# orishu/kraken

Hardware: AMD Instinct MI355X
Metric: metainfo+digest GB/s (device-resident & end-to-end) at 1/2/4/8 MI355X (higher is better)
Workload: dtype u8

## Files before the change

kraken_amd/csrc/sha256_multi.hip:

```cpp
#include <stdlib.h>

#include <atomic>
#include <mutex>
#include <type_traits>

#include "../../include/kraken_hip_internal.h"
#include "kernels.hpp"
#include "knobs.hpp"
#include "device_util.hpp"

namespace krk {

#define KRK_K256                                                                                 \
    0x428a2f98u, 0x71374491u, 0xb5c0fbcfu, 0xe9b5dba5u, 0x3956c25bu, 0x59f111f1u, 0x923f82a4u,     \
        0xab1c5ed5u, 0xd807aa98u, 0x12835b01u, 0x243185beu, 0x550c7dc3u, 0x72be5d74u, 0x80deb1feu, \
        0x9bdc06a7u, 0xc19bf174u, 0xe49b69c1u, 0xefbe4786u, 0x0fc19dc6u, 0x240ca1ccu, 0x2de92c6fu, \
        0x4a7484aau, 0x5cb0a9dcu, 0x76f988dau, 0x983e5152u, 0xa831c66du, 0xb00327c8u, 0xbf597fc7u, \
        0xc6e00bf3u, 0xd5a79147u, 0x06ca6351u, 0x14292967u, 0x27b70a85u, 0x2e1b2138u, 0x4d2c6dfcu, \
        0x53380d13u, 0x650a7354u, 0x766a0abbu, 0x81c2c92eu, 0x92722c85u, 0xa2bfe8a1u, 0xa81a664bu, \
        0xc24b8b70u, 0xc76c51a3u, 0xd192e819u, 0xd6990624u, 0xf40e3585u, 0x106aa070u, 0x19a4c116u, \
        0x1e376c08u, 0x2748774cu, 0x34b0bcb5u, 0x391c0cb3u, 0x4ed8aa4au, 0x5b9cca4fu, 0x682e6ff3u, \
        0x748f82eeu, 0x78a5636fu, 0x84c87814u, 0x8cc70208u, 0x90befffau, 0xa4506cebu, 0xbef9a3f7u, \
        0xc67178f2u

// ... 216 lines not shown
            const int i = 4 * q + t;
            uint32_t wi;
            if (i < 16) {
                wi = w[i];
            } else {
                const uint32_t w15 = w[(i - 15) & 15], w2 = w[(i - 2) & 15];
                const uint32_t s0 = xor3(rotr(w15, 7), rotr(w15, 18), w15 >> 3);
                const uint32_t s1 = xor3(rotr(w2, 17), rotr(w2, 19), w2 >> 10);
                wi = w[i & 15] + s0 + w[(i - 7) & 15] + s1;
                w[i & 15] = wi;
            }
            kw[t] = wi + K[i];
        }
        *reinterpret_cast<u32x4*>(lds + base + 256 * q) = u32x4{kw[0], kw[1], kw[2], kw[3]};
    }
}

template <int kNs, int kStep, bool kNoLoad = false>
__device__ __forceinline__ void produce_step(const ShaJob& job, uint32_t b, uint32_t ob, uint32_t nb,
                                             uint32_t col, uint32_t* lds, const u32x4 use[kRaw],
                                             u32x4 next[kRaw], uint64_t safe, uint32_t& passed) {
    const bool act = b < nb;
    if (act) {
        while (passed + kNs / kStep < b / kStep + 2) {
            __syncthreads();
            ++passed;
        }
    }
    if (kNoLoad) {
#pragma unroll
        for (int c = 0; c < kRaw; ++c) next[c] = u32x4{b, col, (uint32_t)c, b ^ col};
    } else {
        fetch(job, ob + 2 * kStep, next, safe);
    }
    const uint32_t base = kw_base((ob / kStep) % (kNs / kStep), col);
    if (act) build<kNs>(job, ob, use, base, lds);
}

#define KRK_SHA_ROUND(A, B, C, D, E, F, G, HK, KWN, NE, NA, NH)                  \
    "v_alignbit_b32 %[r6], %[" #E "], %[" #E "], 6\n\t"                        \
    "v_alignbit_b32 %[r11], %[" #E "], %[" #E "], 11\n\t"                      \
    "v_alignbit_b32 %[r25], %[" #E "], %[" #E "], 25\n\t"                      \
    "v_bitop3_b32 %[ch], %[" #E "], %[" #F "], %[" #G "] bitop3:0xca\n\t"     \
    "v_bitop3_b32 %[r6], %[r6], %[r11], %[r25] bitop3:0x96\n\t"                \
    "v_alignbit_b32 %[q2], %[" #A "], %[" #A "], 2\n\t"                        \
    "v_add3_u32 %[t1], %[" #HK "], %[r6], %[ch]\n\t"                           \
    "v_alignbit_b32 %[q13], %[" #A "], %[" #A "], 13\n\t"                      \
    "v_add_u32_e32 %[" #NE "], %[" #D "], %[t1]\n\t"                           \
    "v_alignbit_b32 %[q22], %[" #A "], %[" #A "], 22\n\t"                      \
    "v_bitop3_b32 %[mj], %[" #A "], %[" #B "], %[" #C "] bitop3:0xe8\n\t"     \
    "v_bitop3_b32 %[q2], %[q2], %[q13], %[q22] bitop3:0x96\n\t"                \
    "v_add_u32_e32 %[" #NH "], %[" #G "], %[" #KWN "]\n\t"                     \
    "v_add3_u32 %[" #NA "], %[t1], %[q2], %[mj]\n\t"

__device__ __forceinline__ void sha_quad(uint32_t& a, uint32_t& b, uint32_t& c, uint32_t& d, uint32_t& e,
                                         uint32_t& f, uint32_t& g, uint32_t& hk, uint32_t k1, uint32_t k2,
                                         uint32_t k3, uint32_t k4, uint32_t& h_last) {
    uint32_t r6, r11, r25, ch, q2, t1, q13, q22, mj;
    uint32_t e1, e2, e3, e4, a1, a2, a3, a4, h1, h2, h3, h4;
    asm volatile(KRK_SHA_ROUND(a, b, c, d, e, f, g, hk, k1, e1, a1, h1)
                 KRK_SHA_ROUND(a1, a, b, c, e1, e, f, h1, k2, e2, a2, h2)
                 KRK_SHA_ROUND(a2, a1, a, b, e2, e1, e, h2, k3, e3, a3, h3)
                 KRK_SHA_ROUND(a3, a2, a1, a, e3, e2, e1, h3, k4, e4, a4, h4)
                 : [r6] "=&v"(r6), [r11] "=&v"(r11), [r25] "=&v"(r25), [ch] "=&v"(ch), [q2] "=&v"(q2),
                   [t1] "=&v"(t1), [q13] "=&v"(q13), [q22] "=&v"(q22), [mj] "=&v"(mj), [e1] "=&v"(e1),
                   [e2] "=&v"(e2), [e3] "=&v"(e3), [e4] "=&v"(e4), [a1] "=&v"(a1), [a2] "=&v"(a2),
                   [a3] "=&v"(a3), [a4] "=&v"(a4), [h1] "=&v"(h1), [h2] "=&v"(h2), [h3] "=&v"(h3),
                   [h4] "=&v"(h4)
                 : [a] "v"(a), [b] "v"(b), [c] "v"(c), [d] "v"(d), [e] "v"(e), [f] "v"(f), [g] "v"(g),
                   [hk] "v"(hk), [k1] "v"(k1), [k2] "v"(k2), [k3] "v"(k3), [k4] "v"(k4));
    h_last = e1;
    a = a4; b = a3; c = a2; d = a1;
    e = e4; f = e3; g = e2;
    hk = h4;
}
#undef KRK_SHA_ROUND

__device__ __forceinline__ void rounds(uint32_t h[8], const uint32_t* lds, int slot, uint32_t lane,
                                       const u32x4& k0, const u32x4& k1) {
    uint32_t a = h[0], b = h[1], c = h[2], d = h[3], e = h[4], f = h[5], g = h[6];
    uint32_t hk = h[7] + k0[0], hl = 0;
    u32x4 kw = k0, nkw = k1, nnkw = k1;
#pragma unroll
    for (int q = 0; q < 16; ++q) {
        if (q + 2 < 16) nnkw = *reinterpret_cast<const u32x4*>(lds + kw_index(slot, q + 2, lane));
        sha_quad(a, b, c, d, e, f, g, hk, kw[1], kw[2], kw[3], q + 1 < 16 ? nkw[0] : 0u, hl);
        kw = nkw;
        nkw = nnkw;
    }
    h[0] += a; h[1] += b; h[2] += c; h[3] += d; h[4] += e; h[5] += f; h[6] += g; h[7] += hl;
}

__device__ __forceinline__ u32x4 kw_quad(const uint32_t* lds, int slot, int q, uint32_t lane) {
    return *reinterpret_cast<const u32x4*>(lds + kw_index(slot, q, lane));
}

__device__ __forceinline__ bool two_lane_is_e(uint32_t lane) { return (lane >> 3) & 1; }
__device__ __forceinline__ uint32_t two_lane_stream(uint32_t lane) {
    return (lane >> 4) * 8 + (two_lane_is_e(lane) ? 7 - (lane & 7) : (lane & 7));
}

#define KRK_SHA2_ROUND(X0, X1, X2, NX, WN)                                              \
    "v_add_u32_dpp %[p], %[" #X1 "], %[z] row_mirror row_mask:0xf bank_mask:0xf\n\t"    \
    "v_alignbit_b32 %[t1], %[" #X0 "], %[" #X0 "], %[r1]\n\t"                          \
    "v_alignbit_b32 %[t2], %[" #X0 "], %[" #X0 "], %[r2]\n\t"                          \
    "v_alignbit_b32 %[t3], %[" #X0 "], %[" #X0 "], %[r3]\n\t"                          \
    "v_bitop3_b32 %[k], %[" #X0 "], %[" #X1 "], %[ma] bitop3:0x2d\n\t"                 \
    "v_bitop3_b32 %[t1], %[t1], %[t2], %[t3] bitop3:0x96\n\t"                          \
    "v_bitop3_b32 %[k], %[k], %[" #X2 "], %[" #X1 "] bitop3:0xca\n\t"                  \
    "v_xad_u32 %[z], %[" #X2 "], %[ma], %[" #WN "]\n\t"                                \
    "v_add3_u32 %[" #NX "], %[t1], %[k], %[p]\n\t"

struct TwoLaneConst {
    uint32_t r1, r2, r3, ma;
};

#define KRK_SHA2_OPERANDS                                                                             \
    : [t1] "=&v"(t1), [t2] "=&v"(t2), [t3] "=&v"(t3), [k] "=&v"(kk), [p] "=&v"(p), [z] "+v"(z),       \
      [R0] "+v"(R0), [R1] "+v"(R1), [R2] "+v"(R2), [R3] "+v"(R3)
#define KRK_SHA2_CONSTS [r1] "v"(c.r1), [r2] "v"(c.r2), [r3] "v"(c.r3), [ma] "v"(c.ma)

#define KRK_SHA8_ROUND(X0, X1, X2, NX, WN) KRK_SHA8_ROUND_(X0, X1, X2, NX, "%[" #WN "]")
#define KRK_SHA8_ROUND_(X0, X1, X2, NX, W)                                                   \
    "v_alignbit_b32 %[t1], %[" #X0 "], %[" #X0 "], %[r1]\n\t"                               \
    "v_bitop3_b32 %[k], %[" #X0 "], %[" #X1 "], %[ma] bitop3:0x2d\n\t"                      \
    "v_bitop3_b32 %[k], %[k], %[" #X2 "], %[" #X1 "] bitop3:0xca\n\t"                       \
    "v_xor_b32_dpp %[t2], %[t1], %[t1] quad_perm:[1,2,0,3] row_mask:0xf bank_mask:0xf\n\t"  \
    "v_xor_b32_dpp %[t2], %[t1], %[t2] quad_perm:[2,0,1,3] row_mask:0xf bank_mask:0xf\n\t"  \
    "v_add_u32_dpp %[p], %[" #X1 "], %[z] row_ror:8 row_mask:0xf bank_mask:0xf\n\t"          \
    "v_xad_u32 %[z], %[" #X2 "], %[ma], " W "\n\t"                                          \
    "v_add3_u32 %[" #NX "], %[t2], %[k], %[p]\n\t"
#define KRK_SHA8_OPERANDS                                                                    \
    : [t1] "=&v"(t1), [t2] "=&v"(t2), [k] "=&v"(kk), [p] "=&v"(p), [z] "+v"(z), [R0] "+v"(R0), \
      [R1] "+v"(R1), [R2] "+v"(R2), [R3] "+v"(R3)
#define KRK_SHA8_CONSTS [r1] "v"(c.r1), [ma] "v"(c.ma)

constexpr int kHeld8 = 9;
#define KRK_SHA8_RD(Q0, Q1, BASE, OFF, Q) \
    "ds_read_b128 v[" #Q0 ":" #Q1 "], %[" #BASE "] offset:%[" #OFF "]+" #Q "*1024\n\t"
#define KRK_SHA8_QT(W1, W2, W3, W4, B)                                                \
    KRK_SHA8_ROUND_(R2, R1, R0, R3, #W1) B KRK_SHA8_ROUND_(R3, R2, R1, R0, #W2)      \
    KRK_SHA8_ROUND_(R0, R3, R2, R1, #W3) KRK_SHA8_ROUND_(R1, R0, R3, R2, #W4)
#define KRK_SHA8_BURST_A                                                                          \
    "s_waitcnt lgkmcnt(0)\n\t"                                                                    \
    KRK_SHA8_RD(100, 103, cb, co, 9) KRK_SHA8_RD(104, 107, cb, co, 10) KRK_SHA8_RD(108, 111, cb, co, 11) \
    KRK_SHA8_RD(112, 115, cb, co, 12) KRK_SHA8_RD(116, 119, cb, co, 13) KRK_SHA8_RD(120, 123, cb, co, 14) \
    KRK_SHA8_RD(124, 127, cb, co, 15) KRK_SHA8_RD(64, 67, nb, no, 0)
#define KRK_SHA8_BURST_B                                                                          \
    "s_waitcnt lgkmcnt(0)\n\t"                                                                    \
    KRK_SHA8_RD(68, 71, nb, no, 1) KRK_SHA8_RD(72, 75, nb, no, 2) KRK_SHA8_RD(76, 79, nb, no, 3)   \
    KRK_SHA8_RD(80, 83, nb, no, 4) KRK_SHA8_RD(84, 87, nb, no, 5) KRK_SHA8_RD(88, 91, nb, no, 6)   \
    KRK_SHA8_RD(92, 95, nb, no, 7) KRK_SHA8_RD(96, 99, nb, no, 8)

template <uint32_t kCurOff, uint32_t kNxtOff>
__device__ __forceinline__ void block8p(uint32_t& R0, uint32_t& R1, uint32_t& R2, uint32_t& R3, uint32_t& z,
                                        uint32_t hE[4], uint32_t hA[4], uint32_t mineE, uint32_t mineA,
                                        uint32_t i, uint32_t cur, uint32_t nxt, const TwoLaneConst& c,
                                        u32x4 k[kHeld8]) {
    uint32_t t1, t2, kk, p, cc, dd, c2;
    asm volatile(KRK_SHA8_QT(v67, v68, v69, v70, KRK_SHA8_BURST_A)
                 KRK_SHA8_QT(v71, v72, v73, v74, "")
                 KRK_SHA8_QT(v75, v76, v77, v78, "")
                 KRK_SHA8_QT(v79, v80, v81, v82, "")
                 KRK_SHA8_QT(v83, v84, v85, v86, "")
                 KRK_SHA8_QT(v87, v88, v89, v90, "")
                 KRK_SHA8_QT(v91, v92, v93, v94, "")
                 KRK_SHA8_QT(v95, v96, v97, v98, "")
                 KRK_SHA8_QT(v99, v100, v101, v102, KRK_SHA8_BURST_B)
                 KRK_SHA8_QT(v103, v104, v105, v106, "")
                 KRK_SHA8_QT(v107, v108, v109, v110, "")
                 KRK_SHA8_QT(v111, v112, v113, v114, "")
                 KRK_SHA8_QT(v115, v116, v117, v118, "")
                 KRK_SHA8_QT(v119, v120, v121, v122, "")
                 KRK_SHA8_QT(v123, v124, v125, v126, "")
                 KRK_SHA8_ROUND_(R2, R1, R0, R3, "v127")
                 KRK_SHA8_ROUND_(R3, R2, R1, R0, "v64")
                 "v_sub_u32_e32 %[cc], %[a0], %[e0]\n\t"
                 "v_sub_u32_e32 %[dd], %[a1], %[e1]\n\t"
                 "v_add_u32_e32 %[R0], %[e0], %[R0]\n\t"
                 "v_add_u32_e32 %[R3], %[e1], %[R3]\n\t"
                 "v_mov_b32_dpp %[c2], %[cc] row_ror:8 row_mask:0xf bank_mask:0xf\n\t"
                 "v_add_u32_dpp %[z], %[dd], %[z] row_ror:8 row_mask:0xf bank_mask:0xf\n\t"
                 "v_add_u32_e32 %[R2], %[e2], %[R2]\n\t"
                 "v_add_u32_e32 %[R1], %[e3], %[R1]\n\t"
                 "v_add_u32_e32 %[z], %[e3], %[z]\n\t"
                 "v_cmp_lt_u32_e32 vcc, %[i], %[mineE]\n\t"
                 "v_cndmask_b32_e32 %[e0], %[e0], %[R0], vcc\n\t"
                 "v_cndmask_b32_e32 %[e1], %[e1], %[R3], vcc\n\t"
                 "v_cndmask_b32_e32 %[e2], %[e2], %[R2], vcc\n\t"
                 "v_cndmask_b32_e32 %[e3], %[e3], %[R1], vcc\n\t"
                 KRK_SHA8_ROUND_(R0, R3, R2, R1, "v65")
                 "v_add_u32_e32 %[z], %[c2], %[z]\n\t"
                 KRK_SHA8_ROUND_(R1, R0, R3, R2, "v66")
                 "v_sub_u32_e32 %[z], %[z], %[a1]\n\t"
                 "v_add_u32_e32 %[R0], %[a0], %[R0]\n\t"
                 "v_add_u32_e32 %[R3], %[a1], %[R3]\n\t"
                 "v_add_u32_e32 %[R2], %[a2], %[R2]\n\t"
                 "v_add_u32_e32 %[R1], %[a3], %[R1]\n\t"
                 "v_cmp_lt_u32_e32 vcc, %[i], %[mineA]\n\t"
                 "v_cndmask_b32_e32 %[a0], %[a0], %[R0], vcc\n\t"
                 "v_cndmask_b32_e32 %[a1], %[a1], %[R3], vcc\n\t"
                 "v_cndmask_b32_e32 %[a2], %[a2], %[R2], vcc\n\t"
                 "v_cndmask_b32_e32 %[a3], %[a3], %[R1], vcc\n\t"
                 : [t1] "=&v"(t1), [t2] "=&v"(t2), [k] "=&v"(kk), [p] "=&v"(p), [cc] "=&v"(cc), [dd] "=&v"(dd),
                   [c2] "=&v"(c2), [z] "+v"(z),
                   [R0] "+v"(R0), [R1] "+v"(R1), [R2] "+v"(R2), [R3] "+v"(R3), [e0] "+v"(hE[0]),
                   [e1] "+v"(hE[1]), [e2] "+v"(hE[2]), [e3] "+v"(hE[3]), [a0] "+v"(hA[0]), [a1] "+v"(hA[1]),
                   [a2] "+v"(hA[2]), [a3] "+v"(hA[3]),
                   "+{v[64:67]}"(k[0]), "+{v[68:71]}"(k[1]), "+{v[72:75]}"(k[2]), "+{v[76:79]}"(k[3]),
                   "+{v[80:83]}"(k[4]), "+{v[84:87]}"(k[5]), "+{v[88:91]}"(k[6]), "+{v[92:95]}"(k[7]),
                   "+{v[96:99]}"(k[8])
                 : KRK_SHA8_CONSTS, [i] "s"(i), [mineE] "v"(mineE), [mineA] "v"(mineA), [cb] "v"(cur),
                   [nb] "v"(nxt), [co] "n"(kCurOff), [no] "n"(kNxtOff)
                 : "vcc", "memory", "v100", "v101", "v102", "v103", "v104", "v105", "v106", "v107", "v108",
                   "v109", "v110", "v111", "v112", "v113", "v114", "v115", "v116", "v117", "v118", "v119", "v120",
                   "v121", "v122", "v123", "v124", "v125", "v126", "v127");
}
#undef KRK_SHA8_QT
#undef KRK_SHA8_BURST_A
#undef KRK_SHA8_BURST_B
#undef KRK_SHA8_RD

__device__ __forceinline__ void prologue8p(uint32_t& R0, uint32_t& R1, uint32_t& R2, uint32_t& R3, uint32_t& z,
                                           const uint32_t h[4], bool is_e, const TwoLaneConst& c,
                                           const u32x4& k0) {
    {
        uint32_t t1, t2, kk, p;
        asm volatile("v_xad_u32 %[z], %[R1], %[ma], %[w0]\n\t"
                     KRK_SHA8_ROUND(R0, R3, R2, R1, w1)
                     KRK_SHA8_OPERANDS
                     : KRK_SHA8_CONSTS, [w0] "v"(k0[0]), [w1] "v"(k0[1]));
    }
    R1 = is_e ? R1 : h[3];
    {
        uint32_t t1, t2, kk, p;
        asm volatile(KRK_SHA8_ROUND(R1, R0, R3, R2, w2)
                     KRK_SHA8_OPERANDS
                     : KRK_SHA8_CONSTS, [w2] "v"(k0[2]));
    }
    R2 = is_e ? R2 : h[2];
}

constexpr int kAhead2 = 4;
__device__ __forceinline__ void sha2_dodec2(uint32_t& R0, uint32_t& R1, uint32_t& R2, uint32_t& R3, uint32_t& z,
                                            const TwoLaneConst& c, const u32x4& a, const u32x4& b, const u32x4& d,
                                            const u32x4& e) {
    uint32_t t1, t2, t3, kk, p;
    asm volatile(KRK_SHA2_ROUND(R2, R1, R0, R3, w1) KRK_SHA2_ROUND(R3, R2, R1, R0, w2)
                 KRK_SHA2_ROUND(R0, R3, R2, R1, w3) KRK_SHA2_ROUND(R1, R0, R3, R2, w4)
                 KRK_SHA2_ROUND(R2, R1, R0, R3, w5) KRK_SHA2_ROUND(R3, R2, R1, R0, w6)
                 KRK_SHA2_ROUND(R0, R3, R2, R1, w7) KRK_SHA2_ROUND(R1, R0, R3, R2, w8)
                 KRK_SHA2_ROUND(R2, R1, R0, R3, w9) KRK_SHA2_ROUND(R3, R2, R1, R0, w10)
                 KRK_SHA2_ROUND(R0, R3, R2, R1, w11) KRK_SHA2_ROUND(R1, R0, R3, R2, w12)
                 KRK_SHA2_OPERANDS
                 : KRK_SHA2_CONSTS, [w1] "v"(a[3]), [w2] "v"(b[0]), [w3] "v"(b[1]), [w4] "v"(b[2]),
                   [w5] "v"(b[3]), [w6] "v"(d[0]), [w7] "v"(d[1]), [w8] "v"(d[2]), [w9] "v"(d[3]),
                   [w10] "v"(e[0]), [w11] "v"(e[1]), [w12] "v"(e[2]));
    (void)t3;
}

__device__ __forceinline__ void block2p(uint32_t& R0, uint32_t& R1, uint32_t& R2, uint32_t& R3, uint32_t& z,
                                        uint32_t hE[4], uint32_t hA[4], uint32_t mineE, uint32_t mineA,
                                        uint32_t i, const uint32_t* lds, uint32_t cbase, uint32_t nbase,
                                        const TwoLaneConst& c, u32x4 k[kAhead2]) {
    constexpr int kRS = kAhead2 + 1;
    u32x4 wq[kRS];
#pragma unroll
    for (int j = 0; j < kAhead2; ++j) wq[j] = k[j];
    constexpr int RS = kAhead2 + 3;
    u32x4 wr[RS];
#pragma unroll
    for (int j = 0; j < kAhead2; ++j) wr[j] = wq[j];
    auto rd = [&](int q) {
        if (q < 16) wr[q % RS] = *reinterpret_cast<const u32x4*>(lds + cbase + 256 * q);
        else k[q - 16] = *reinterpret_cast<const u32x4*>(lds + nbase + 256 * (q - 16));
    };
#pragma unroll
    for (int j = 0; j < 15; j += 3) {
        rd(j + kAhead2);
        rd(j + kAhead2 + 1);
        rd(j + kAhead2 + 2);
        sha2_dodec2(R0, R1, R2, R3, z, c, wr[j % RS], wr[(j + 1) % RS], wr[(j + 2) % RS], wr[(j + 3) % RS]);
    }
    wq[15 % kRS] = wr[15 % RS];
    k[kAhead2 - 1] = *reinterpret_cast<const u32x4*>(lds + nbase + 256 * (kAhead2 - 1));
    {
        uint32_t t1, t2, t3, kk, p;
        asm volatile(KRK_SHA2_ROUND(R2, R1, R0, R3, w3)
                     KRK_SHA2_ROUND(R3, R2, R1, R0, w4)
                     KRK_SHA2_OPERANDS
                     : KRK_SHA2_CONSTS, [w3] "v"(wq[15 % kRS][3]), [w4] "v"(k[0][0]));
    }
    {
        uint32_t t1, t2, t3, kk, p, cc, dd, c2, w1c;
        asm volatile("v_sub_u32_e32 %[cc], %[a0], %[e0]\n\t"
                     "v_sub_u32_e32 %[dd], %[a1], %[e1]\n\t"
                     "v_add_u32_e32 %[R0], %[e0], %[R0]\n\t"
                     "v_add_u32_e32 %[R3], %[e1], %[R3]\n\t"
                     "v_mov_b32_dpp %[c2], %[cc] row_mirror row_mask:0xf bank_mask:0xf\n\t"
                     "v_add_u32_dpp %[z], %[dd], %[z] row_mirror row_mask:0xf bank_mask:0xf\n\t"
                     "v_add_u32_e32 %[R2], %[e2], %[R2]\n\t"
                     "v_add_u32_e32 %[R1], %[e3], %[R1]\n\t"
                     "v_add_u32_e32 %[z], %[e3], %[z]\n\t"
                     "v_cmp_lt_u32_e32 vcc, %[i], %[mineE]\n\t"
                     "v_cndmask_b32_e32 %[e0], %[e0], %[R0], vcc\n\t"
                     "v_cndmask_b32_e32 %[e1], %[e1], %[R3], vcc\n\t"
                     "v_cndmask_b32_e32 %[e2], %[e2], %[R2], vcc\n\t"
                     "v_cndmask_b32_e32 %[e3], %[e3], %[R1], vcc\n\t"
                     "v_add_u32_e32 %[w1c], %[c2], %[w1]\n\t"
                     KRK_SHA2_ROUND(R0, R3, R2, R1, w1c)
                     KRK_SHA2_ROUND(R1, R0, R3, R2, w2)
                     "v_sub_u32_e32 %[z], %[z], %[a1]\n\t"
                     "v_add_u32_e32 %[R0], %[a0], %[R0]\n\t"
                     "v_add_u32_e32 %[R3], %[a1], %[R3]\n\t"
                     "v_add_u32_e32 %[R2], %[a2], %[R2]\n\t"
                     "v_add_u32_e32 %[R1], %[a3], %[R1]\n\t"
                     "v_cmp_lt_u32_e32 vcc, %[i], %[mineA]\n\t"
                     "v_cndmask_b32_e32 %[a0], %[a0], %[R0], vcc\n\t"
                     "v_cndmask_b32_e32 %[a1], %[a1], %[R3], vcc\n\t"
                     "v_cndmask_b32_e32 %[a2], %[a2], %[R2], vcc\n\t"
                     "v_cndmask_b32_e32 %[a3], %[a3], %[R1], vcc\n\t"
                     : [t1] "=&v"(t1), [t2] "=&v"(t2), [t3] "=&v"(t3), [k] "=&v"(kk), [p] "=&v"(p), [cc] "=&v"(cc),
                       [dd] "=&v"(dd), [c2] "=&v"(c2), [w1c] "=&v"(w1c), [z] "+v"(z),
                       [R0] "+v"(R0), [R1] "+v"(R1), [R2] "+v"(R2), [R3] "+v"(R3), [e0] "+v"(hE[0]),
                       [e1] "+v"(hE[1]), [e2] "+v"(hE[2]), [e3] "+v"(hE[3]), [a0] "+v"(hA[0]), [a1] "+v"(hA[1]),
                       [a2] "+v"(hA[2]), [a3] "+v"(hA[3])
                     : KRK_SHA2_CONSTS, [w1] "v"(k[0][1]), [w2] "v"(k[0][2]), [i] "s"(i), [mineE] "v"(mineE),
                       [mineA] "v"(mineA)
                     : "vcc");
    }
}

__device__ __forceinline__ void prologue2p(uint32_t& R0, uint32_t& R1, uint32_t& R2, uint32_t& R3, uint32_t& z,
                                           const uint32_t h[4], bool is_e, const TwoLaneConst& c,
                                           const u32x4& k0) {
    {
        uint32_t t1, t2, t3, kk, p;
        asm volatile("s_nop 0\n\t"
                     "v_xad_u32 %[z], %[R1], %[ma], %[w0]\n\t"
                     KRK_SHA2_ROUND(R0, R3, R2, R1, w1)
                     KRK_SHA2_OPERANDS
                     : KRK_SHA2_CONSTS, [w0] "v"(k0[0]), [w1] "v"(k0[1]));
    }
    R1 = is_e ? R1 : h[3];
    {
        uint32_t t1, t2, t3, kk, p;
        asm volatile(KRK_SHA2_ROUND(R1, R0, R3, R2, w2)
                     KRK_SHA2_OPERANDS
                     : KRK_SHA2_CONSTS, [w2] "v"(k0[2]));
    }
    R2 = is_e ? R2 : h[2];
}
#undef KRK_SHA2_OPERANDS
#undef KRK_SHA2_CONSTS
#undef KRK_SHA8_OPERANDS
#undef KRK_SHA8_CONSTS

__device__ __forceinline__ uint32_t wave_min(uint32_t v) {
#pragma unroll
    for (int off = 32; off > 0; off >>= 1) v = min(v, (uint32_t)__shfl_xor((int)v, off, 64));
    return __builtin_amdgcn_readfirstlane(v);
}

template <int kTiming, bool kTwo, int kGroups = 1>
__global__ void __launch_bounds__(128 * kGroups)
sha256_ws_kernel(const ShaJob* __restrict__ jobs, uint32_t n_jobs, uint8_t* __restrict__ out_digest,
                 uint32_t* __restrict__ out_state) {
    extern __shared__ __attribute__((aligned(16))) uint32_t ring_all[];
    constexpr int kNs = kTwo ? kSlots2 : kSlots;
    constexpr int kStep = kTwo ? 2 : 1;
// ... 33 lines not shown
            produce_step<kNs, kStep, kTiming == 3>(job, b + kStep, b + kStep + par, nb, col, ring, R1, R0, safe,
                                                   passed);
            produce_step<kNs, kStep, kTiming == 3>(job, b + 2 * kStep, b + 2 * kStep + par, nb, col, ring, R2, R1,
                                                   safe, passed);
        }
        while (passed < (nb + kStep - 1) / kStep) {
            __syncthreads();
            ++passed;
        }
    } else if (kTwo) {
        const bool is_e = two_lane_is_e(lane);
        const uint32_t half = is_e ? 4u : 0u;
        const TwoLaneConst c{is_e ? 6u : 2u, is_e ? 11u : 13u, is_e ? 25u : 22u, is_e ? 0u : ~0u};
        uint32_t h[4];
        if (live && (job.flags & kShaFromState)) {
#pragma unroll
            for (int k = 0; k < 4; ++k) h[k] = out_state[8 * (uint64_t)job.out + half + (is_e ? k : k ^ 2)];
        } else {
#pragma unroll
            for (int k = 0; k < 4; ++k) h[k] = is_e ? job.h[4 + k] : job.h[k ^ 2];
        }
        __builtin_amdgcn_s_setprio(3);
        const uint32_t aoff = is_e ? 0u : uint32_t(kRing2) * kSlotWords;
        const uint32_t base_even = aoff + (lane ^ 15u) * 4, base_odd = aoff + lane * 4;
        const uint32_t einc = is_e ? uint32_t(kSlotWords) : 0u;
        uint32_t vslot = 0, slot = 0;
        u32x4 kq[kAhead2] = {};
        uint32_t hE[4], hA[4];
#pragma unroll
        for (int k = 0; k < 4; ++k) {
            hE[k] = is_e ? h[k] : 0u;
            hA[k] = is_e ? 0u : h[k];
        }
        const uint32_t mineE = is_e ? mine : 0u, mineA = is_e ? 0u : mine;
        uint32_t R0 = h[0], R3 = h[1], R2 = h[2], R1 = h[3], z = 0;
        auto block = [&](uint32_t i, uint32_t cur, uint32_t nxt) {
            block2p(R0, R1, R2, R3, z, hE, hA, mineE, mineA, i, ring, cur, nxt, c, kq);
        };
        if (nb) {
            if (kTiming == 0) __builtin_amdgcn_s_barrier();
            asm volatile("" ::: "memory");
#pragma unroll
            for (int q = 0; q < kAhead2; ++q) kq[q] = *reinterpret_cast<const u32x4*>(ring + base_even + 256 * q);
            prologue2p(R0, R1, R2, R3, z, h, is_e, c, kq[0]);
        }
        for (uint32_t i = 0; i < nb; i += 2) {
            if (i) {
                if (kTiming == 0) __builtin_amdgcn_s_barrier();
                asm volatile("" ::: "memory");
            }
            const uint32_t nslot = slot == kRing2 - 1 ? 0u : slot + 1;
            const uint32_t nvslot = slot == kRing2 - 1 ? 0u : vslot + einc;
            block(i, base_even + vslot, base_odd + vslot);
            if (i + 1 < nb) block(i + 1, base_odd + vslot, base_even + nvslot);
            slot = nslot;
            vslot = nvslot;
        }
#pragma unroll
        for (int k = 0; k < 4; ++k) h[k] = is_e ? hE[k] : hA[k];
        if (live) {
            uint32_t hs[4];
#pragma unroll
            for (int k = 0; k < 4; ++k) hs[k] = is_e ? h[k] : h[k ^ 2];
            if (job.flags & kShaFinal) {
                uint8_t* o = out_digest + 32 * (uint64_t)job.out + 4 * half;
                if ((reinterpret_cast<uintptr_t>(o) & 15) == 0) {
                    reinterpret_cast<uint4*>(o)[0] =
                        make_uint4(bswap(hs[0]), bswap(hs[1]), bswap(hs[2]), bswap(hs[3]));
                } else {
                    for (int k = 0; k < 16; ++k) o[k] = (uint8_t)(hs[k >> 2] >> (24 - 8 * (k & 3)));
                }
            } else {
                uint32_t* o = out_state + 8 * (uint64_t)job.out + half;
#pragma unroll
                for (int k = 0; k < 4; ++k) o[k] = hs[k];
            }
        }
    } else {
        uint32_t h[8];
        if (live && (job.flags & kShaFromState)) {
#pragma unroll
            for (int k = 0; k < 8; ++k) h[k] = out_state[8 * (uint64_t)job.out + k];
        } else {
#pragma unroll
            for (int k = 0; k < 8; ++k) h[k] = job.h[k];
        }
        __builtin_amdgcn_s_setprio(3);
        const uint32_t common = wave_min(live ? mine : ~0u);
        u32x4 k0{}, k1{};
        for (uint32_t i = 0; i < nb; ++i) {
            if (kTiming == 0) __builtin_amdgcn_s_barrier();
            asm volatile("" ::: "memory");
            if (i == 0) {
                k0 = kw_quad(ring, 0, 0, lane);
                k1 = kw_quad(ring, 0, 1, lane);
            }
            uint32_t x[8];
#pragma unroll
            for (int k = 0; k < 8; ++k) x[k] = h[k];
            rounds(x, ring, (int)(i % kSlots), lane, k0, k1);
            if (i + 1 < nb) {
                k0 = kw_quad(ring, (int)((i + 1) % kSlots), 0, lane);
                k1 = kw_quad(ring, (int)((i + 1) % kSlots), 1, lane);
            }
            if (i < common) {
#pragma unroll
                for (int k = 0; k < 8; ++k) h[k] = x[k];
            } else if (i < mine) {
#pragma unroll
                for (int k = 0; k < 8; ++k) h[k] = x[k];
            }
        }
        if (live) {
            if (job.flags & kShaFinal) {
                uint8_t* o = out_digest + 32 * (uint64_t)job.out;
                if ((reinterpret_cast<uintptr_t>(o) & 15) == 0) {
                    reinterpret_cast<uint4*>(o)[0] = make_uint4(bswap(h[0]), bswap(h[1]), bswap(h[2]), bswap(h[3]));
                    reinterpret_cast<uint4*>(o)[1] = make_uint4(bswap(h[4]), bswap(h[5]), bswap(h[6]), bswap(h[7]));
                } else {
                    for (int k = 0; k < 32; ++k) o[k] = (uint8_t)(h[k >> 2] >> (24 - 8 * (k & 3)));
                }
            } else {
                uint32_t* o = out_state + 8 * (uint64_t)job.out;
#pragma unroll
                for (int k = 0; k < 8; ++k) o[k] = h[k];
            }
        }
    }
}

template <int kTiming, int kGroups>
__global__ void __launch_bounds__(128 * kGroups)
sha256_w8_kernel(const ShaJob* __restrict__ jobs, uint32_t n_jobs, uint8_t* __restrict__ out_digest,
                 uint32_t* __restrict__ out_state) {
    extern __shared__ __attribute__((aligned(16))) uint32_t ring_all[];
    constexpr int kStep8 = 8, kRing8 = 3, kNs = kStep8 * kRing8;
    constexpr uint32_t kPer = 8;
    constexpr uint32_t kRingWords = uint32_t(kRing8 + 1) * kSlotWords + kOnesPad8;
    const uint32_t lane = threadIdx.x & 63;
    const uint32_t wave = threadIdx.x >> 6;
    const bool producer = wave < (uint32_t)kGroups;
    const uint32_t grp = wave % kGroups;
    uint32_t* ring = ring_all + grp * kRingWords;
    const uint32_t sbase = blockIdx.x * kPer * kGroups;
    const uint32_t quad = (lane >> 2) & 3;
    const uint32_t me = producer ? (lane & 7) : (lane >> 4) * 2 + (quad & 1);
    const uint32_t j = sbase + grp * kPer + me;
    const bool live = j < n_jobs;
    ShaJob job{};
    if (live) job = jobs[j];
    const uint32_t mine = live ? job_blocks(job) : 0u;
    const uint32_t nb = workgroup_blocks<kGroups>(jobs, n_jobs, sbase, kPer, me, grp, mine);

    if (producer && kTiming == 1) return;
    if (producer) {
#pragma unroll
        for (int q = 0; q < 16; ++q) *reinterpret_cast<u32x4*>(ring + kw_index(kRing8, q, lane)) = u32x4{1u, 1u, 1u, 1u};
        *reinterpret_cast<u32x4*>(ring + (kRing8 + 1) * kSlotWords + lane * 4) = u32x4{1u, 1u, 1u, 1u};
        u32x4 R0[kRaw], R1[kRaw], R2[kRaw];
        const uint64_t safe = reinterpret_cast<uint64_t>(jobs);
        const uint32_t par = lane >> 3;
        uint32_t passed = 0;
        fetch(job, par, R0, safe);
        fetch(job, par + kStep8, R1, safe);
        for (uint32_t b = 0; b < nb; b += 3 * kStep8) {
            produce_step<kNs, kStep8>(job, b, b + par, nb, lane, ring, R0, R2, safe, passed);
            produce_step<kNs, kStep8>(job, b + kStep8, b + kStep8 + par, nb, lane, ring, R1, R0, safe, passed);
            produce_step<kNs, kStep8>(job, b + 2 * kStep8, b + 2 * kStep8 + par, nb, lane, ring, R2, R1, safe, passed);
        }
        while (passed < (nb + kStep8 - 1) / kStep8) {
            __syncthreads();
            ++passed;
        }
        return;
    }
    const bool is_e = quad < 2;
    const uint32_t pos = lane & 3;
    const uint32_t half = is_e ? 4u : 0u;
    const uint32_t r1 = is_e ? (pos == 1 ? 11u : pos == 2 ? 25u : 6u) : (pos == 1 ? 13u : pos == 2 ? 22u : 2u);
    const TwoLaneConst c{r1, 0u, 0u, is_e ? 0u : ~0u};
    uint32_t h[4];
    if (live && (job.flags & kShaFromState)) {
#pragma unroll
        for (int k = 0; k < 4; ++k) h[k] = out_state[8 * (uint64_t)job.out + half + (is_e ? k : k ^ 2)];
    } else {
#pragma unroll
        for (int k = 0; k < 4; ++k) h[k] = is_e ? job.h[4 + k] : job.h[k ^ 2];
    }
    __builtin_amdgcn_s_setprio(3);
    const uint32_t lbase = is_e ? me * 4u : uint32_t(kRing8) * kSlotWords + 32u;
    const uint32_t binc = 32u, sinc = is_e ? uint32_t(kSlotWords) : 0u;
    uint32_t voff = 0, vslot = 0, slot = 0;
    const uint32_t lbyte = (uint32_t)(uintptr_t)(__attribute__((address_space(3))) uint32_t*)ring + 4u * lbase;
    u32x4 kq[kHeld8] = {};
    uint32_t hE[4], hA[4];
#pragma unroll
    for (int k = 0; k < 4; ++k) {
        hE[k] = is_e ? h[k] : 0u;
        hA[k] = is_e ? 0u : h[k];
    }
    const uint32_t mineE = is_e ? mine : 0u, mineA = is_e ? 0u : mine;
    uint32_t R0 = h[0], R3 = h[1], R2 = h[2], R1 = h[3], z = 0;
    constexpr uint32_t kU = 4;
    static_assert(kStep8 % kU == 0, "blocks per iteration divide a step");
    if (nb) {
        if (kTiming == 0) __builtin_amdgcn_s_barrier();
        asm volatile("" ::: "memory");
#pragma unroll
        for (int q = 0; q < kHeld8; ++q) kq[q] = *reinterpret_cast<const u32x4*>(ring + lbase + 256 * q);
        prologue8p(R0, R1, R2, R3, z, h, is_e, c, kq[0]);
    }
    for (uint32_t i = 0; i < nb; i += kU) {
        const uint32_t jj = i & (kStep8 - 1);
        if (jj == 0 && i) {
            if (kTiming == 0) __builtin_amdgcn_s_barrier();
            asm volatile("" ::: "memory");
        }
        const bool last = jj == kStep8 - kU;
        const uint32_t nvslot = slot == kRing8 - 1 ? 0u : vslot + sinc;
        const uint32_t cur = lbyte + 4u * voff;
        voff = last ? nvslot : voff + kU * binc;
        const uint32_t nxt = lbyte + 4u * voff;
        constexpr uint32_t kB = 4u * binc;
        [&] {
            block8p<0, kB>(R0, R1, R2, R3, z, hE, hA, mineE, mineA, i, cur, cur, c, kq);
            if (i + 1 < nb) block8p<kB, 2 * kB>(R0, R1, R2, R3, z, hE, hA, mineE, mineA, i + 1, cur, cur, c, kq);
            if (i + 2 < nb) block8p<2 * kB, 3 * kB>(R0, R1, R2, R3, z, hE, hA, mineE, mineA, i + 2, cur, cur, c, kq);
            if (i + 3 < nb) block8p<3 * kB, 0>(R0, R1, R2, R3, z, hE, hA, mineE, mineA, i + 3, cur, nxt, c, kq);
        }();
        if (last) {
            slot = slot == kRing8 - 1 ? 0u : slot + 1;
            vslot = nvslot;
        }
    }
    asm volatile("s_waitcnt lgkmcnt(0)"
                 : "+{v[64:67]}"(kq[0]), "+{v[68:71]}"(kq[1]), "+{v[72:75]}"(kq[2]), "+{v[76:79]}"(kq[3]),
                   "+{v[80:83]}"(kq[4]), "+{v[84:87]}"(kq[5]), "+{v[88:91]}"(kq[6]), "+{v[92:95]}"(kq[7]),
                   "+{v[96:99]}"(kq[8])
                 :
                 : "memory");
#pragma unroll
    for (int k = 0; k < 4; ++k) h[k] = is_e ? hE[k] : hA[k];
    if (live && pos == 0) {
        uint32_t hs[4];
#pragma unroll
        for (int k = 0; k < 4; ++k) hs[k] = is_e ? h[k] : h[k ^ 2];
        if (job.flags & kShaFinal) {
            uint8_t* o = out_digest + 32 * (uint64_t)job.out + 4 * half;
            if ((reinterpret_cast<uintptr_t>(o) & 15) == 0) {
                reinterpret_cast<uint4*>(o)[0] = make_uint4(bswap(hs[0]), bswap(hs[1]), bswap(hs[2]), bswap(hs[3]));
            } else {
                for (int k = 0; k < 16; ++k) o[k] = (uint8_t)(hs[k >> 2] >> (24 - 8 * (k & 3)));
            }
        } else {
            uint32_t* o = out_state + 8 * (uint64_t)job.out + half;
#pragma unroll
            for (int k = 0; k < 4; ++k) o[k] = hs[k];
        }
    }
}

using ShaLaunch = hipError_t (*)(const ShaJob*, uint32_t, uint8_t*, uint32_t*, hipStream_t);

template <auto kKernel, size_t kPairLds, uint32_t kPairStreams, int kPairs>
static hipError_t launch_pairs(const ShaJob* jobs, uint32_t n_jobs, uint8_t* out_digest, uint32_t* out_state,
                               hipStream_t s) {
    constexpr size_t lds = kPairLds * kPairs;
    constexpr uint32_t per = kPairStreams * kPairs;
    static std::once_flag once;
    static hipError_t attr_err = hipSuccess;
    std::call_once(once, [] {
        attr_err = hipFuncSetAttribute(reinterpret_cast<const void*>(kKernel),
                                       hipFuncAttributeMaxDynamicSharedMemorySize, (int)lds);
    });
    if (attr_err != hipSuccess) return attr_err;
    if (const hipError_t p_ = launch_precheck(); p_ != hipSuccess) return p_;
    hipLaunchKernelGGL(kKernel, dim3((n_jobs + per - 1) / per), dim3(128 * kPairs), lds, s, jobs, n_jobs, out_digest,
                       out_state);
    return hipGetLastError();
}

template <int kLanes, int kPairs, int kTiming>
static hipError_t launch_lanes(const ShaJob* jobs, uint32_t n_jobs, uint8_t* out_digest, uint32_t* out_state,
                               hipStream_t s) {
    static_assert(kLanes == 1 || kLanes == 2 || kLanes == 8, "lanes a stream");
    if constexpr (kLanes == 8) {
        return launch_pairs<&sha256_w8_kernel<kTiming, kPairs>, (4 * kSlotWords + kOnesPad8) * 4, 8, kPairs>(
            jobs, n_jobs, out_digest, out_state, s);
    } else {
        constexpr bool kTwo = kLanes == 2;
        return launch_pairs<&sha256_ws_kernel<kTiming, kTwo, kPairs>, size_t(kTwo ? kRing2 + 1 : kSlots) * kSlotWords * 4,
                            kTwo ? 32 : 64, kPairs>(jobs, n_jobs, out_digest, out_state, s);
    }
}

#ifdef KRK_DIAG
static hipError_t launch_multi(const ShaJob* jobs, uint32_t n_jobs, uint8_t* out_digest, uint32_t* out_state,
                                  hipStream_t s) {
    if (const hipError_t p_ = launch_precheck(); p_ != hipSuccess) return p_;
    hipLaunchKernelGGL(sha256_multi_kernel, dim3((n_jobs + 63) / 64), dim3(64), 0, s, jobs, n_jobs, out_digest,
                       out_state);
    return hipGetLastError();
}
#endif

struct ShaPlan {
    int id, lanes, pairs, timing;
    ShaLaunch launch;
};
template <int kLanes, int kPairs, int kTiming = 0>
constexpr ShaPlan sha_plan_row(int id) {
    return {id, kLanes, kPairs, kTiming, &launch_lanes<kLanes, kPairs, kTiming>};
}
constexpr ShaPlan kShaPlans[] = {
    sha_plan_row<1, 1>(KRK_SHA_PLAN_1LANE),
    sha_plan_row<2, 1>(KRK_SHA_PLAN_2LANE),
    sha_plan_row<1, 2>(KRK_SHA_PLAN_1LANE_2PAIR),
    sha_plan_row<2, 2>(KRK_SHA_PLAN_2LANE_2PAIR),
    sha_plan_row<8, 1>(KRK_SHA_PLAN_8LANE),
    sha_plan_row<8, 2>(KRK_SHA_PLAN_8LANE_2PAIR),
#ifdef KRK_DIAG
    {100, 1, 1, 0, &launch_multi},
    sha_plan_row<1, 1>(101),
    sha_plan_row<1, 1, 1>(102),
    sha_plan_row<2, 1>(103),
    sha_plan_row<2, 1, 1>(104),
    sha_plan_row<1, 1, 2>(105),
    sha_plan_row<2, 1, 2>(106),
    sha_plan_row<2, 1, 3>(107),
    sha_plan_row<8, 1, 1>(108),
#endif
};

static const ShaPlan* find_plan(int id) {
    for (const ShaPlan& p : kShaPlans)
        if (p.id == id) return &p;
    return nullptr;
}

bool sha_plan_valid(int p) { return p == KRK_SHA_PLAN_AUTO || find_plan(p); }

static std::atomic<int> g_sha_plan{-1};

static int sha_plan() {
    int p = g_sha_plan.load(std::memory_order_relaxed);
    if (p >= 0) return p;
    const char* e = KRK_AB_ENV("KRK_SHA_PLAN");
    int want = e ? atoi(e) : KRK_SHA_PLAN_AUTO;
    if (!sha_plan_valid(want)) want = KRK_SHA_PLAN_AUTO;
    int expect = -1;
    g_sha_plan.compare_exchange_strong(expect, want);
    return g_sha_plan.load(std::memory_order_relaxed);
}

void set_sha_plan(int p) { g_sha_plan.store(p, std::memory_order_relaxed); }

static uint32_t device_cus() {
    static uint32_t n = [] {
        int dev = 0, cus = 256;
        if (hipGetDevice(&dev) == hipSuccess) {
            hipDeviceProp_t p;
            if (hipGetDeviceProperties(&p, dev) == hipSuccess && p.multiProcessorCount > 0) cus = p.multiProcessorCount;
        }
        return (uint32_t)cus;
    }();
    return n;
}

static int auto_plan(uint32_t n_jobs) {
    if (n_jobs <= device_cus() * 16u) return KRK_SHA_PLAN_8LANE;
    if (n_jobs <= device_cus() * 32u) return KRK_SHA_PLAN_2LANE;
    return n_jobs <= device_cus() * 64u ? KRK_SHA_PLAN_2LANE_2PAIR : KRK_SHA_PLAN_1LANE_2PAIR;
}

static int resolve_plan(uint32_t n_jobs) {
    const int p = sha_plan();
    return p == KRK_SHA_PLAN_AUTO ? auto_plan(n_jobs) : p;
}

int sha_plan_for(uint32_t n_jobs) { return resolve_plan(n_jobs); }

int sha_lanes_for(uint32_t n_jobs) {
    const ShaPlan* p = find_plan(resolve_plan(n_jobs));
    return p ? p->lanes : 1;
}

hipError_t launch_sha256(const ShaJob* jobs, uint32_t n_jobs, uint8_t* out_digest,
                         uint32_t* out_state, hipStream_t s) {
    if (!n_jobs) return hipSuccess;
    return launch_sha256_plan(resolve_plan(n_jobs), jobs, n_jobs, out_digest, out_state, s);
}

hipError_t launch_sha256_plan(int plan, const ShaJob* jobs, uint32_t n_jobs, uint8_t* out_digest,
                              uint32_t* out_state, hipStream_t s) {
    if (!n_jobs) return hipSuccess;
    t_launch_plan = plan;
    t_launch_units = n_jobs;
    const ShaPlan* p = find_plan(plan);
    return p ? p->launch(jobs, n_jobs, out_digest, out_state, s) : hipErrorInvalidValue;
}

__global__ void __launch_bounds__(256) digest_scatter_kernel(const uint8_t* __restrict__ rec, uint32_t n,
                                                             uint8_t* __restrict__ digests) {
    const uint32_t t = blockIdx.x * blockDim.x + threadIdx.x;
    if (t >= n * 32) return;
    const uint8_t* r = rec + 36 * (t / 32);
    const uint32_t idx = (uint32_t)r[0] | ((uint32_t)r[1] << 8) | ((uint32_t)r[2] << 16) | ((uint32_t)r[3] << 24);
    digests[32ull * idx + t % 32] = r[4 + t % 32];
}

hipError_t launch_digest_scatter(const uint8_t* rec, uint32_t n, uint8_t* digests, hipStream_t s) {
    if (!n) return hipSuccess;
    if (const hipError_t p_ = launch_precheck(); p_ != hipSuccess) return p_;
    hipLaunchKernelGGL(digest_scatter_kernel, dim3((n * 32 + 255) / 256), dim3(256), 0, s, rec, n, digests);
    return hipGetLastError();
}

}
```

Measured before the change: 59.93.

## Add full-step fast path for 8-lane SHA with constant masks and scalar compares

Splits the 8-lane SHA-256 block loop into a full-step path and a tail. In the full step every lane still has blocks left, so the per-block commit masks become compile-time constants and the ring offsets are computed once per step. The tail keeps the per-block compare, now done as scalar uicmp producing an SGPR mask instead of a v_cmp into vcc inside the asm. It also adds a diagnostic timing mode (plan 109) that skips the boundary bookkeeping, and larger unrolled code may raise instruction-cache pressure.

```diff
diff --git a/kraken_amd/csrc/sha256_multi.hip b/kraken_amd/csrc/sha256_multi.hip
--- a/kraken_amd/csrc/sha256_multi.hip
+++ b/kraken_amd/csrc/sha256_multi.hip
@@ -392,70 +392,81 @@
     KRK_SHA8_RD(80, 83, nb, no, 4) KRK_SHA8_RD(84, 87, nb, no, 5) KRK_SHA8_RD(88, 91, nb, no, 6)   \
     KRK_SHA8_RD(92, 95, nb, no, 7) KRK_SHA8_RD(96, 99, nb, no, 8)
 
-template <uint32_t kCurOff, uint32_t kNxtOff>
+#define KRK_SHA8_SNAP(H, M)                                              \
+    "v_cndmask_b32_e64 %[" #H "0], %[" #H "0], %[R0], %[" #M "]\n\t"     \
+    "v_cndmask_b32_e64 %[" #H "1], %[" #H "1], %[R3], %[" #M "]\n\t"     \
+    "v_cndmask_b32_e64 %[" #H "2], %[" #H "2], %[R2], %[" #M "]\n\t"     \
+    "v_cndmask_b32_e64 %[" #H "3], %[" #H "3], %[R1], %[" #M "]\n\t"
+#define KRK_SHA8_F1                                                              \
+    "v_sub_u32_e32 %[cc], %[a0], %[e0]\n\t"                                      \
+    "v_sub_u32_e32 %[dd], %[a1], %[e1]\n\t"                                      \
+    "v_add_u32_e32 %[R0], %[e0], %[R0]\n\t"                                      \
+    "v_add_u32_e32 %[R3], %[e1], %[R3]\n\t"                                      \
+    "v_mov_b32_dpp %[c2], %[cc] row_ror:8 row_mask:0xf bank_mask:0xf\n\t"        \
+    "v_add_u32_dpp %[z], %[dd], %[z] row_ror:8 row_mask:0xf bank_mask:0xf\n\t"   \
+    "v_add_u32_e32 %[R2], %[e2], %[R2]\n\t"                                      \
+    "v_add_u32_e32 %[R1], %[e3], %[R1]\n\t"                                      \
+    "v_add_u32_e32 %[z], %[e3], %[z]\n\t"                                        \
+    KRK_SHA8_SNAP(e, mE)
+#define KRK_SHA8_F2 "v_add_u32_e32 %[z], %[c2], %[z]\n\t"
+#define KRK_SHA8_F3                                 \
+    "v_sub_u32_e32 %[z], %[z], %[a1]\n\t"           \
+    "v_add_u32_e32 %[R0], %[a0], %[R0]\n\t"         \
+    "v_add_u32_e32 %[R3], %[a1], %[R3]\n\t"         \
+    "v_add_u32_e32 %[R2], %[a2], %[R2]\n\t"         \
+    "v_add_u32_e32 %[R1], %[a3], %[R1]\n\t"         \
+    KRK_SHA8_SNAP(a, mA)
+#define KRK_SHA8_BLOCK(F1, F2, F3)                                \
+    KRK_SHA8_QT(v67, v68, v69, v70, KRK_SHA8_BURST_A)             \
+    KRK_SHA8_QT(v71, v72, v73, v74, "")                           \
+    KRK_SHA8_QT(v75, v76, v77, v78, "")                           \
+    KRK_SHA8_QT(v79, v80, v81, v82, "")                           \
+    KRK_SHA8_QT(v83, v84, v85, v86, "")                           \
+    KRK_SHA8_QT(v87, v88, v89, v90, "")                           \
+    KRK_SHA8_QT(v91, v92, v93, v94, "")                           \
+    KRK_SHA8_QT(v95, v96, v97, v98, "")                           \
+    KRK_SHA8_QT(v99, v100, v101, v102, KRK_SHA8_BURST_B)          \
+    KRK_SHA8_QT(v103, v104, v105, v106, "")                       \
+    KRK_SHA8_QT(v107, v108, v109, v110, "")                       \
+    KRK_SHA8_QT(v111, v112, v113, v114, "")                       \
+    KRK_SHA8_QT(v115, v116, v117, v118, "")                       \
+    KRK_SHA8_QT(v119, v120, v121, v122, "")                       \
+    KRK_SHA8_QT(v123, v124, v125, v126, "")                       \
+    KRK_SHA8_ROUND_(R2, R1, R0, R3, "v127")                       \
+    KRK_SHA8_ROUND_(R3, R2, R1, R0, "v64")                        \
+    F1 KRK_SHA8_ROUND_(R0, R3, R2, R1, "v65") F2 KRK_SHA8_ROUND_(R1, R0, R3, R2, "v66") F3
+#define KRK_SHA8_BLOCK_OPERANDS                                                                              \
+    : [t1] "=&v"(t1), [t2] "=&v"(t2), [k] "=&v"(kk), [p] "=&v"(p), [cc] "=&v"(cc), [dd] "=&v"(dd),           \
+      [c2] "=&v"(c2), [z] "+v"(z),                                                                           \
+      [R0] "+v"(R0), [R1] "+v"(R1), [R2] "+v"(R2), [R3] "+v"(R3), [e0] "+v"(hE[0]),                          \
+      [e1] "+v"(hE[1]), [e2] "+v"(hE[2]), [e3] "+v"(hE[3]), [a0] "+v"(hA[0]), [a1] "+v"(hA[1]),              \
+      [a2] "+v"(hA[2]), [a3] "+v"(hA[3]),                                                                    \
+                            \
+      "+{v[64:67]}"(k[0]), "+{v[68:71]}"(k[1]), "+{v[72:75]}"(k[2]), "+{v[76:79]}"(k[3]),                    \
+      "+{v[80:83]}"(k[4]), "+{v[84:87]}"(k[5]), "+{v[88:91]}"(k[6]), "+{v[92:95]}"(k[7]),                    \
+      "+{v[96:99]}"(k[8])                                                                                    \
+    : KRK_SHA8_CONSTS, [mE] "s"(mE), [mA] "s"(mA), [cb] "v"(cur),                                            \
+      [nb] "v"(nxt), [co] "n"(kCurOff), [no] "n"(kNxtOff)                                                    \
+    : "memory", "v100", "v101", "v102", "v103", "v104", "v105", "v106", "v107", "v108",                      \
+      "v109", "v110", "v111", "v112", "v113", "v114", "v115", "v116", "v117", "v118", "v119", "v120",        \
+      "v121", "v122", "v123", "v124", "v125", "v126", "v127"
+template <uint32_t kCurOff, uint32_t kNxtOff, bool kBoundary>
 __device__ __forceinline__ void block8p(uint32_t& R0, uint32_t& R1, uint32_t& R2, uint32_t& R3, uint32_t& z,
-                                        uint32_t hE[4], uint32_t hA[4], uint32_t mineE, uint32_t mineA,
-                                        uint32_t i, uint32_t cur, uint32_t nxt, const TwoLaneConst& c,
-                                        u32x4 k[kHeld8]) {
+                                        uint32_t hE[4], uint32_t hA[4], uint64_t mE, uint64_t mA, uint32_t cur,
+                                        uint32_t nxt, const TwoLaneConst& c, u32x4 k[kHeld8]) {
     uint32_t t1, t2, kk, p, cc, dd, c2;
-    asm volatile(KRK_SHA8_QT(v67, v68, v69, v70, KRK_SHA8_BURST_A)
-                 KRK_SHA8_QT(v71, v72, v73, v74, "")
-                 KRK_SHA8_QT(v75, v76, v77, v78, "")
-                 KRK_SHA8_QT(v79, v80, v81, v82, "")
-                 KRK_SHA8_QT(v83, v84, v85, v86, "")
-                 KRK_SHA8_QT(v87, v88, v89, v90, "")
-                 KRK_SHA8_QT(v91, v92, v93, v94, "")
-                 KRK_SHA8_QT(v95, v96, v97, v98, "")
-                 KRK_SHA8_QT(v99, v100, v101, v102, KRK_SHA8_BURST_B)
-                 KRK_SHA8_QT(v103, v104, v105, v106, "")
-                 KRK_SHA8_QT(v107, v108, v109, v110, "")
-                 KRK_SHA8_QT(v111, v112, v113, v114, "")
-                 KRK_SHA8_QT(v115, v116, v117, v118, "")
-                 KRK_SHA8_QT(v119, v120, v121, v122, "")
-                 KRK_SHA8_QT(v123, v124, v125, v126, "")
-                 KRK_SHA8_ROUND_(R2, R1, R0, R3, "v127")
-                 KRK_SHA8_ROUND_(R3, R2, R1, R0, "v64")
-                 "v_sub_u32_e32 %[cc], %[a0], %[e0]\n\t"
-                 "v_sub_u32_e32 %[dd], %[a1], %[e1]\n\t"
-                 "v_add_u32_e32 %[R0], %[e0], %[R0]\n\t"
-                 "v_add_u32_e32 %[R3], %[e1], %[R3]\n\t"
-                 "v_mov_b32_dpp %[c2], %[cc] row_ror:8 row_mask:0xf bank_mask:0xf\n\t"
-                 "v_add_u32_dpp %[z], %[dd], %[z] row_ror:8 row_mask:0xf bank_mask:0xf\n\t"
-                 "v_add_u32_e32 %[R2], %[e2], %[R2]\n\t"
-                 "v_add_u32_e32 %[R1], %[e3], %[R1]\n\t"
-                 "v_add_u32_e32 %[z], %[e3], %[z]\n\t"
-                 "v_cmp_lt_u32_e32 vcc, %[i], %[mineE]\n\t"
-                 "v_cndmask_b32_e32 %[e0], %[e0], %[R0], vcc\n\t"
-                 "v_cndmask_b32_e32 %[e1], %[e1], %[R3], vcc\n\t"
-                 "v_cndmask_b32_e32 %[e2], %[e2], %[R2], vcc\n\t"
-                 "v_cndmask_b32_e32 %[e3], %[e3], %[R1], vcc\n\t"
-                 KRK_SHA8_ROUND_(R0, R3, R2, R1, "v65")
-                 "v_add_u32_e32 %[z], %[c2], %[z]\n\t"
-                 KRK_SHA8_ROUND_(R1, R0, R3, R2, "v66")
-                 "v_sub_u32_e32 %[z], %[z], %[a1]\n\t"
-                 "v_add_u32_e32 %[R0], %[a0], %[R0]\n\t"
-                 "v_add_u32_e32 %[R3], %[a1], %[R3]\n\t"
-                 "v_add_u32_e32 %[R2], %[a2], %[R2]\n\t"
-                 "v_add_u32_e32 %[R1], %[a3], %[R1]\n\t"
-                 "v_cmp_lt_u32_e32 vcc, %[i], %[mineA]\n\t"
-                 "v_cndmask_b32_e32 %[a0], %[a0], %[R0], vcc\n\t"
-                 "v_cndmask_b32_e32 %[a1], %[a1], %[R3], vcc\n\t"
-                 "v_cndmask_b32_e32 %[a2], %[a2], %[R2], vcc\n\t"
-                 "v_cndmask_b32_e32 %[a3], %[a3], %[R1], vcc\n\t"
-                 : [t1] "=&v"(t1), [t2] "=&v"(t2), [k] "=&v"(kk), [p] "=&v"(p), [cc] "=&v"(cc), [dd] "=&v"(dd),
-                   [c2] "=&v"(c2), [z] "+v"(z),
-                   [R0] "+v"(R0), [R1] "+v"(R1), [R2] "+v"(R2), [R3] "+v"(R3), [e0] "+v"(hE[0]),
-                   [e1] "+v"(hE[1]), [e2] "+v"(hE[2]), [e3] "+v"(hE[3]), [a0] "+v"(hA[0]), [a1] "+v"(hA[1]),
-                   [a2] "+v"(hA[2]), [a3] "+v"(hA[3]),
-                   "+{v[64:67]}"(k[0]), "+{v[68:71]}"(k[1]), "+{v[72:75]}"(k[2]), "+{v[76:79]}"(k[3]),
-                   "+{v[80:83]}"(k[4]), "+{v[84:87]}"(k[5]), "+{v[88:91]}"(k[6]), "+{v[92:95]}"(k[7]),
-                   "+{v[96:99]}"(k[8])
-                 : KRK_SHA8_CONSTS, [i] "s"(i), [mineE] "v"(mineE), [mineA] "v"(mineA), [cb] "v"(cur),
-                   [nb] "v"(nxt), [co] "n"(kCurOff), [no] "n"(kNxtOff)
-                 : "vcc", "memory", "v100", "v101", "v102", "v103", "v104", "v105", "v106", "v107", "v108",
-                   "v109", "v110", "v111", "v112", "v113", "v114", "v115", "v116", "v117", "v118", "v119", "v120",
-                   "v121", "v122", "v123", "v124", "v125", "v126", "v127");
-}
+    if constexpr (kBoundary) {
+        asm volatile(KRK_SHA8_BLOCK(KRK_SHA8_F1, KRK_SHA8_F2, KRK_SHA8_F3) KRK_SHA8_BLOCK_OPERANDS);
+    } else {
+        asm volatile(KRK_SHA8_BLOCK("", "", "") KRK_SHA8_BLOCK_OPERANDS);
+    }
+}
+#undef KRK_SHA8_BLOCK_OPERANDS
+#undef KRK_SHA8_BLOCK
+#undef KRK_SHA8_F3
+#undef KRK_SHA8_F2
+#undef KRK_SHA8_F1
+#undef KRK_SHA8_SNAP
 #undef KRK_SHA8_QT
 #undef KRK_SHA8_BURST_A
 #undef KRK_SHA8_BURST_B
@@ -795,7 +806,8 @@
     const uint32_t mine = live ? job_blocks(job) : 0u;
     const uint32_t nb = workgroup_blocks<kGroups>(jobs, n_jobs, sbase, kPer, me, grp, mine);
 
-    if (producer && kTiming == 1) return;
+    constexpr bool kAlone = kTiming == 1 || kTiming == 4;
+    if (producer && kAlone) return;
     if (producer) {
 #pragma unroll
         for (int q = 0; q < 16; ++q) *reinterpret_cast<u32x4*>(ring + kw_index(kRing8, q, lane)) = u32x4{1u, 1u, 1u, 1u};
@@ -847,16 +859,45 @@
     constexpr uint32_t kU = 4;
     static_assert(kStep8 % kU == 0, "blocks per iteration divide a step");
     if (nb) {
-        if (kTiming == 0) __builtin_amdgcn_s_barrier();
+        if (!kAlone) __builtin_amdgcn_s_barrier();
         asm volatile("" ::: "memory");
 #pragma unroll
         for (int q = 0; q < kHeld8; ++q) kq[q] = *reinterpret_cast<const u32x4*>(ring + lbase + 256 * q);
         prologue8p(R0, R1, R2, R3, z, h, is_e, c, kq[0]);
     }
-    for (uint32_t i = 0; i < nb; i += kU) {
+    constexpr uint32_t kB = 4u * binc;
+    constexpr bool kBnd = kTiming != 4;
+    uint32_t i = 0;
+    {
+        constexpr uint32_t kSlotBytes = 4u * uint32_t(kSlotWords);
+        constexpr uint64_t kMaskE = 0x00ff00ff00ff00ffull, kMaskA = ~kMaskE;
+        const uint32_t emask = is_e ? ~0u : 0u;
+        const uint32_t nfull = min(nb, wave_min(live ? mine : ~0u)) & ~uint32_t(kStep8 - 1);
+        uint32_t soff = 0;
+        for (; i < nfull; i += kStep8) {
+            if (i) {
+                if (!kAlone) __builtin_amdgcn_s_barrier();
+                asm volatile("" ::: "memory");
+            }
+            const uint32_t noff = soff == (kRing8 - 1) * kSlotBytes ? 0u : soff + kSlotBytes;
+            const uint32_t cur = lbyte + (soff & emask), nxt = lbyte + (noff & emask);
+            block8p<0, kB, kBnd>(R0, R1, R2, R3, z, hE, hA, kMaskE, kMaskA, cur, cur, c, kq);
+            block8p<kB, 2 * kB, kBnd>(R0, R1, R2, R3, z, hE, hA, kMaskE, kMaskA, cur, cur, c, kq);
+            block8p<2 * kB, 3 * kB, kBnd>(R0, R1, R2, R3, z, hE, hA, kMaskE, kMaskA, cur, cur, c, kq);
+            block8p<3 * kB, 4 * kB, kBnd>(R0, R1, R2, R3, z, hE, hA, kMaskE, kMaskA, cur, cur, c, kq);
+            block8p<4 * kB, 5 * kB, kBnd>(R0, R1, R2, R3, z, hE, hA, kMaskE, kMaskA, cur, cur, c, kq);
+            block8p<5 * kB, 6 * kB, kBnd>(R0, R1, R2, R3, z, hE, hA, kMaskE, kMaskA, cur, cur, c, kq);
+            block8p<6 * kB, 7 * kB, kBnd>(R0, R1, R2, R3, z, hE, hA, kMaskE, kMaskA, cur, cur, c, kq);
+            block8p<7 * kB, 0, kBnd>(R0, R1, R2, R3, z, hE, hA, kMaskE, kMaskA, cur, nxt, c, kq);
+            soff = noff;
+        }
+        slot = soff / kSlotBytes;
+        voff = vslot = (soff / 4u) & emask;
+    }
+    for (; i < nb; i += kU) {
         const uint32_t jj = i & (kStep8 - 1);
         if (jj == 0 && i) {
-            if (kTiming == 0) __builtin_amdgcn_s_barrier();
+            if (!kAlone) __builtin_amdgcn_s_barrier();
             asm volatile("" ::: "memory");
         }
         const bool last = jj == kStep8 - kU;
@@ -864,13 +905,14 @@
         const uint32_t cur = lbyte + 4u * voff;
         voff = last ? nvslot : voff + kU * binc;
         const uint32_t nxt = lbyte + 4u * voff;
-        constexpr uint32_t kB = 4u * binc;
+#define KRK_M8(U) __builtin_amdgcn_uicmp(i + U, mineE, 36), __builtin_amdgcn_uicmp(i + U, mineA, 36)
         [&] {
-            block8p<0, kB>(R0, R1, R2, R3, z, hE, hA, mineE, mineA, i, cur, cur, c, kq);
-            if (i + 1 < nb) block8p<kB, 2 * kB>(R0, R1, R2, R3, z, hE, hA, mineE, mineA, i + 1, cur, cur, c, kq);
-            if (i + 2 < nb) block8p<2 * kB, 3 * kB>(R0, R1, R2, R3, z, hE, hA, mineE, mineA, i + 2, cur, cur, c, kq);
-            if (i + 3 < nb) block8p<3 * kB, 0>(R0, R1, R2, R3, z, hE, hA, mineE, mineA, i + 3, cur, nxt, c, kq);
+            block8p<0, kB, kBnd>(R0, R1, R2, R3, z, hE, hA, KRK_M8(0), cur, cur, c, kq);
+            if (i + 1 < nb) block8p<kB, 2 * kB, kBnd>(R0, R1, R2, R3, z, hE, hA, KRK_M8(1), cur, cur, c, kq);
+            if (i + 2 < nb) block8p<2 * kB, 3 * kB, kBnd>(R0, R1, R2, R3, z, hE, hA, KRK_M8(2), cur, cur, c, kq);
+            if (i + 3 < nb) block8p<3 * kB, 0, kBnd>(R0, R1, R2, R3, z, hE, hA, KRK_M8(3), cur, nxt, c, kq);
         }();
+#undef KRK_M8
         if (last) {
             slot = slot == kRing8 - 1 ? 0u : slot + 1;
             vslot = nvslot;
@@ -972,6 +1014,7 @@
     sha_plan_row<2, 1, 2>(106),
     sha_plan_row<2, 1, 3>(107),
     sha_plan_row<8, 1, 1>(108),
+    sha_plan_row<8, 1, 4>(109),
 #endif
 };
 
```

Result: faster. 60.87, median of 6 (+1.6%).
